# chem-rano/eigensolvers

Hardware: AMD Instinct MI355X
Metric: fp64 CSR SpMV GB/s (fused shift y = sigma*x - H x) (higher is better)
Workload: dtype f64; 1 GPU; random-sparse Hermitian CSR N=10000000 nnz/row~64 (BASELINE metric config), row-partitioned over 1 GPU(s); N=10000000, nnz=650007472, nnz_row_arg=64, kernel_variant=auto:column-window-blocked(workgroup), generator_seed=7, comm=auto

## Files before the change

### eigensolvers_amd/csrc/common.h

```cpp
#pragma once
#include <hip/hip_runtime.h>
#include <stdint.h>
#include <stdio.h>
#include <stdlib.h>
#include <string.h>
#include "../../include/hipeig.h"

#define HIPEIG_WAVE 64
#define HIPEIG_BLOCK 256
#define HIPEIG_MAX_PARTIALS 2048
#define HIPEIG_MAX_COLS 16
#define HIPEIG_WIDE_PARTIALS 32768
#define HIPEIG_GATHER_MAX_CHUNKS 4
#define HIPEIG_SLOT_DOUBLES 16
#define HIPEIG_MAX_RANKS 64

struct GatherLayout {
  int32_t nranks, nchunks;
  int64_t h;
  int64_t cbase[HIPEIG_GATHER_MAX_CHUNKS + 1];
  __host__ __device__ int64_t cstride(int c) const { return h + (c == nchunks - 1 ? HIPEIG_SLOT_DOUBLES : 0); }
  __host__ __device__ int64_t pos(int rank, int64_t i) const {
    int c = (int)(i / h);
    if (c >= nchunks) c = nchunks - 1;
// ... 86 lines not shown
  double* mr_ws;
  int64_t mr_ws_n;
  int64_t mr_ws_doubles;
  hipGraphExec_t mr_graph;
  void* mr_graph_key;
  size_t mr_graph_key_bytes;
  int use_graph;
  MinresState* d_mr_state;
  MinresState* h_mr_state;
  void* comm;
  void* loop;
  int nranks, rank;
  int collectives;
  int64_t mr_collectives;
  double* x_full;
  int64_t x_full_n;
  int64_t* row_counts;
  double* blk_ws;
  size_t blk_ws_doubles;
  double* xb_full;
  int64_t xb_full_n;
  double* mrb_ws;
  int64_t mrb_ws_n;
  MinresState* d_mrb_state;
  MinresState* h_mrb_state;
  double* mrbz_ws;
  int64_t mrbz_ws_n;
  int overlap;
  double* ytmp;
  int64_t ytmp_n;
  int gather_chunks;
  hipEvent_t ev_chunk[HIPEIG_GATHER_MAX_CHUNKS];
  unsigned* d_counters;
  double* d_group_partials;
  int phase_timing;
  hipEvent_t ev_ph[8];
  hipEvent_t ev_stage;
  hipEvent_t ev_slot[16];
  hipStream_t arn_stream[16];
  hipEvent_t ev_arn_in[16];
  int arn_nstreams;
  double* d_arn_ws;
  unsigned* d_arn_cnt;
  void* h_arn_items;
  void* d_arn_items;
  struct DirectComm* direct;
  int gather_backend;
  int allreduce_backend;
  int exchange_off;
  double* ms_ws;
  int64_t ms_ws_doubles;
  void* h_ms_state;
  double* lf_ws;
  int64_t lf_ws_doubles;
  void* h_lf_state;
  struct LfPoolEntry* lf_pool;
  int lf_pool_n, lf_pool_cap;
  int64_t lf_pool_bytes;
};

struct LfPoolEntry {
  double* p;
  size_t bytes;
};
void hipeig_lf_pool_clear(hipeig_ctx* c);
void arnoldi_release(hipeig_ctx* c);

struct BlockedLayout {
  uint32_t* idx;
  double* val;
  uint32_t* off;
  int32_t nunits, nwin, wbits, rw;
  int32_t wgs_per_sweep;
  int32_t csplit;
  int32_t binbits, align;
  int64_t slots;
  int32_t state;
};

static inline size_t blocked_lds_bytes(const BlockedLayout& L, int acc_per_row) {
  return (size_t)L.rw * acc_per_row * sizeof(double) + ((size_t)L.nwin + 2) * sizeof(uint32_t);
}

struct SweepGrid { int wgs, launches; };
static inline SweepGrid blocked_grid(const BlockedLayout& L, int units_per_wg = 1) {
  const int64_t total = L.csplit > 1 ? (int64_t)L.nunits * L.csplit : ((int64_t)L.nunits + units_per_wg - 1) / units_per_wg;
  int64_t g = (L.csplit > 1 || total < L.wgs_per_sweep) ? total : L.wgs_per_sweep;
  if (g < 1) g = 1;
  if (g > HIPEIG_MAX_PARTIALS) g = HIPEIG_MAX_PARTIALS;
  return SweepGrid{(int)g, (int)((total + g - 1) / g)};
}

enum : unsigned {
  BIN_LANE_MAJOR = 1,
  BIN_UNIT_BATCH = 2,
  BIN_GROUP_ALIGN = 4,
  BIN_WIN_BATCH = 8,
  BIN_UNCACHED = 16,
};

struct hipeig_csr {
  int64_t nrows, ncols, nnz, row_offset;
  int32_t* d_rowptr;
  int32_t* d_col;
  double* d_val;
  int32_t* d_row_blocks;
  int32_t n_row_blocks;
  BlockedLayout t;
  int32_t t_prefetch;
  BlockedLayout w;
  BlockedLayout p;
  BlockedLayout b[3];
  double* d_dense;
  int64_t dense_ld;
  int64_t dense_bytes;
  int32_t dense_grid_vec, dense_grid_blk;
  int32_t last_pair_fused;
  int reproducible;
  double absrow_max;
  int32_t block_variant;
  int32_t last_block_variant, last_block_k;
  int64_t gather_len;
  GatherLayout gl;
  RankRows rank_rows;
  int variant;
  int last_variant;
  int last_launches;
  int lanes_per_row;
  int64_t col_stride;
  int64_t bytes;
};

static inline int layout_slot(int K) { return K == 4 ? 0 : K == 8 ? 1 : 2; }

int hipeig_build_binned(hipeig_ctx* c, hipeig_csr* A, const BlockedLayout& geom, unsigned policy, BlockedLayout* out);
void hipeig_free_layout(BlockedLayout* L);

int hipeig_dense_refusal(const hipeig_ctx* c, const hipeig_csr* A);
int hipeig_dense_reserve(hipeig_ctx* c, hipeig_csr* A);
int hipeig_dense_grid(const hipeig_csr* A, int rows_per_wg);
void hipeig_dense_free(hipeig_csr* A);

int hipeig_sync_checked(hipeig_ctx* c);

int hipeig_comm_setup_rows(hipeig_ctx* ctx, int64_t nrows_local, GatherLayout* gl_out);
int hipeig_allreduce_sum(hipeig_ctx* ctx, double* d_buf, int count);
int hipeig_allgather_x(hipeig_ctx* ctx, const GatherLayout& gl, const double* x_local, int64_t n_local,
                       const double** x_full_out);
int hipeig_allgather_f64(hipeig_ctx* ctx, const double* send, double* recv, size_t count);
int hipeig_allgather_x_begin(hipeig_ctx* ctx, const GatherLayout& gl, const double* x_local, int64_t n_local);
int hipeig_allgather_x_wait_chunk(hipeig_ctx* ctx, const GatherLayout& gl, int chunk);
int hipeig_allgather_block(hipeig_ctx* ctx, const GatherLayout& gl, int K, const double* xb_local, int64_t n_local,
                           const double** xb_full_out);
double* hipeig_gather_slot(hipeig_ctx* ctx, const GatherLayout& gl);

__host__ __device__ __forceinline__ double mul_rn(double a, double b) {
#pragma clang fp contract(off)
  return a * b;
}
__host__ __device__ __forceinline__ double add_rn(double a, double b) {
#pragma clang fp contract(off)
  return a + b;
}

__device__ __forceinline__ double wave_reduce_sum(double v) {
#pragma unroll
  for (int off = 32; off > 0; off >>= 1) v += __shfl_down(v, off, 64);
  return v;
}

// ... 102 lines not shown
```

### eigensolvers_amd/csrc/spmv.hip

```cpp
#include <vector>
#include "sweep_launch.h"

static int build_tcoow_layout(hipeig_ctx* c, hipeig_csr* A, int pair);

struct AxpyEpilogue {
  double a_self, a_sum;
  const double* __restrict__ xl;
  double* __restrict__ y;
  __device__ __forceinline__ void row(int64_t r, double sum, double& acc) const {
    const double t = (a_self == 0.0) ? 0.0 : mul_rn(a_self, xl[r]);
    y[r] = add_rn(t, mul_rn(a_sum, sum));
  }
};

__global__ void __launch_bounds__(HIPEIG_BLOCK)
spmv_stream_kernel(CsrView A, const double* __restrict__ x, AxpyEpilogue epi) {
  __shared__ double prod[SPMV_NNZ_PER_BLOCK];
  double acc = 0.0;
  csr_stream_sweep(A, x, epi, acc, prod);
}

__global__ void __launch_bounds__(HIPEIG_BLOCK)
spmv_vector_kernel(CsrView A, const double* __restrict__ x, AxpyEpilogue epi) {
  double acc = 0.0;
  csr_vector_sweep(A, x, epi, acc);
}

__global__ void __launch_bounds__(HIPEIG_BLOCK)
spmv_tcoo_kernel(TcooView T, const double* __restrict__ x, AxpyEpilogue epi) {
  extern __shared__ double tcoo_lds[];
  double acc = 0.0;
  tcoo_sweep(T, x, epi, acc, tcoo_lds);
}

template <int FIXED>
__global__ void __launch_bounds__(TCOOW_THREADS)
spmv_tcoow_kernel(TcooView T, const double* __restrict__ x, AxpyEpilogue epi) {
  extern __shared__ double tcoo_lds[];
  __shared__ double red16[16];
  double acc = 0.0;
  tcoo_wg_sweep<AxpyEpilogue, FIXED>(T, x, epi, acc, tcoo_lds, red16);
}

__global__ void __launch_bounds__(HIPEIG_BLOCK)
spmv_dense_kernel(DenseView D, const double* __restrict__ x, AxpyEpilogue epi) {
  double acc = 0.0;
  dense_row_sweep(D, x, epi, acc);
}

struct PairEpilogue {
  double ar, ai, as;
  const double* __restrict__ xr;
  const double* __restrict__ xi;
  double* __restrict__ yr;
  double* __restrict__ yi;
  __device__ __forceinline__ void row2(int64_t r, double sr, double si, double& acc) const {
    const double vr = xr[r], vi = xi[r];
    const double tr = add_rn(mul_rn(ar, vr), mul_rn(as, sr));
    const double ti = add_rn(mul_rn(ar, vi), mul_rn(as, si));
    yr[r] = fma(-ai, vi, tr);
    yi[r] = fma(ai, vr, ti);
  }
};

__global__ void __launch_bounds__(TCOOW_THREADS)
spmv_tcoow_pair_kernel(TcooView T, const double* __restrict__ xpair, PairEpilogue epi) {
  extern __shared__ double tcoo_lds[];
  double acc = 0.0;
  tcoo_wg_sweep<PairEpilogue, 0, 1>(T, xpair, epi, acc, tcoo_lds, nullptr);
}

__global__ void __launch_bounds__(HIPEIG_BLOCK)
pair_pack_kernel(int64_t n, const double* __restrict__ xr, const double* __restrict__ xi, double2* __restrict__ xp) {
  const int64_t stride = (int64_t)gridDim.x * blockDim.x;
  for (int64_t i = (int64_t)blockIdx.x * blockDim.x + threadIdx.x; i < n; i += stride) xp[i] = make_double2(xr[i], xi[i]);
}

__global__ void __launch_bounds__(HIPEIG_BLOCK) absmax_kernel(const double* __restrict__ x, int64_t n, double* __restrict__ partials) {
  __shared__ double lds[16];
  double m = 0.0;
  const int64_t stride = (int64_t)gridDim.x * blockDim.x;
  for (int64_t i = (int64_t)blockIdx.x * blockDim.x + threadIdx.x; i < n; i += stride) {
    const double v = fabs(x[i]);
    m = (v > m || v != v) ? v : m;
// ... 3 lines not shown
}

__global__ void __launch_bounds__(HIPEIG_BLOCK)
rowabs_max_kernel(const int32_t* __restrict__ rowptr, const double* __restrict__ val, int64_t nrows, double* __restrict__ partials) {
  __shared__ double lds[16];
  const int lane = threadIdx.x & 63;
  const int64_t wave = ((int64_t)blockIdx.x * blockDim.x + threadIdx.x) >> 6;
  const int64_t nwaves = ((int64_t)gridDim.x * blockDim.x) >> 6;
  double m = 0.0;
  for (int64_t r = wave; r < nrows; r += nwaves) {
    double a = 0.0;
    for (int p = rowptr[r] + lane; p < rowptr[r + 1]; p += 64) a += fabs(val[p]);
    a = wave_reduce_sum(a);
    a = __shfl(a, 0, 64);
    m = fmax(m, a);
  }
  m = block_max_all(m, lds);
  if (threadIdx.x == 0) partials[blockIdx.x] = m;
}

__global__ void __launch_bounds__(HIPEIG_BLOCK) absmax_gathered_kernel(const double* __restrict__ x, GatherLayout gl, RankRows rows,
                                                                       double* __restrict__ partials) {
  __shared__ double lds[16];
  double m = 0.0;
  const int64_t stride = (int64_t)gridDim.x * blockDim.x, n = gl.total();
  for (int64_t p = (int64_t)blockIdx.x * blockDim.x + threadIdx.x; p < n; p += stride) {
    int k = 0;
    while (k + 1 < gl.nchunks && p >= gl.cbase[k + 1]) ++k;
    const int64_t q = p - gl.cbase[k], cs = gl.cstride(k);
    const int r = (int)(q / cs);
    const int64_t i = q - (int64_t)r * cs;
    if (i >= gl.h || (int64_t)k * gl.h + i >= rows.n[r]) continue;
    const double v = fabs(x[p]);
    m = (v > m || v != v) ? v : m;
  }
  m = block_max_all(m, lds);
  if (threadIdx.x == 0) partials[blockIdx.x] = m;
}

#define HIPEIG_FX_AREA (4 * HIPEIG_WIDE_PARTIALS)
int hipeig_fixed_prepare(hipeig_ctx* c, const hipeig_csr* A, const double* xg, TcooView* t) {
  const int g = grid_for(A->gather_len, 8);
  double* area = c->d_partials + HIPEIG_FX_AREA;
  if (A->col_stride > 0)
    hipLaunchKernelGGL(absmax_gathered_kernel, dim3(g), dim3(HIPEIG_BLOCK), 0, c->stream, xg, A->gl, A->rank_rows, area);
  else
    hipLaunchKernelGGL(absmax_kernel, dim3(g), dim3(HIPEIG_BLOCK), 0, c->stream, xg, A->gather_len, area);
  t->fx_xmax = area; t->fx_count = g; t->fx_bound = A->absrow_max;
  return 0;
}

__global__ void __launch_bounds__(HIPEIG_BLOCK)
spmv_tcoow_combine_kernel(const double* __restrict__ parts, int nparts, int64_t stride, int64_t nrows, AxpyEpilogue epi) {
  double acc = 0.0;
  tcoow_combine_sweep(parts, nparts, stride, nrows, epi, acc);
}

static auto spmv_launcher(hipeig_ctx* c, const SweepPlan& p, const AxpyEpilogue& epi) {
  const CsrView view = p.view;
  const DenseView dview = p.dview;
  return [=](auto v, auto f, int grid, int threads, size_t lds, const TcooView& tv, const double* xg, int) {
    constexpr int V = decltype(v)::value;
    const dim3 g(grid), t(threads);
    if constexpr (V == 6) hipLaunchKernelGGL(spmv_dense_kernel, g, t, lds, c->stream, dview, xg, epi);
    else if constexpr (V == 5) hipLaunchKernelGGL(spmv_tcoow_combine_kernel, g, t, lds, c->stream, tv.raw_out, tv.part_base, tv.part_stride, tv.nrows, epi);
    else if constexpr (V == 4) hipLaunchKernelGGL(spmv_tcoow_kernel<decltype(f)::value>, g, t, lds, c->stream, tv, xg, epi);
    else if constexpr (V == 3) hipLaunchKernelGGL(spmv_tcoo_kernel, g, t, lds, c->stream, tv, xg, epi);
    else if constexpr (V == 2) hipLaunchKernelGGL(spmv_stream_kernel, g, t, lds, c->stream, view, xg, epi);
    else hipLaunchKernelGGL(spmv_vector_kernel, g, t, lds, c->stream, view, xg, epi);
  };
}

TcooView hipeig_tcoo_view(const hipeig_csr* A, const BlockedLayout& L) {
  TcooView t;
  t.idx = L.idx; t.val = L.val; t.off = L.off;
  t.nunits = L.nunits; t.nwin = L.nwin; t.wbits = L.wbits; t.rw = L.rw;
  t.unit_begin = 0;
  t.prefetch = (&L == &A->t) ? A->t_prefetch : 0;
  t.ablate = 0;
  if (const char* e = getenv("HIPEIG_TCOO_ABLATE")) t.ablate = atoi(e);
  t.nrows = A->nrows;
  t.gather_len = A->gather_len;
  t.nrun = 0; t.yinit = nullptr; t.raw_out = nullptr;
  t.csplit = 1; t.part_base = 0; t.part_stride = 0;
  t.fx_xmax = nullptr; t.fx_count = 0; t.fx_bound = 0.0;
  return t;
}

CsrView hipeig_csr_view(const hipeig_csr* A) {
  CsrView v;
  v.rowptr = A->d_rowptr;
  v.col = A->d_col;
  v.val = A->d_val;
  v.row_blocks = A->d_row_blocks;
  v.n_row_blocks = A->n_row_blocks;
  v.nrows = A->nrows;
  v.group = A->lanes_per_row;
  return v;
}

SweepGrid hipeig_sweep_grid(const hipeig_csr* A, int variant) {
  if (variant == 6) return SweepGrid{hipeig_dense_grid(A, DENSE_ROWS_PER_WAVE * (HIPEIG_BLOCK / HIPEIG_WAVE)), 1};
  if (variant == 4 || variant == 5) return blocked_grid(A->w);
  if (variant == 3) return blocked_grid(A->t, 4);
  int64_t g = A->n_row_blocks;
  if (variant == 1) {
    const int64_t groups_per_block = HIPEIG_BLOCK / A->lanes_per_row;
    g = (A->nrows + groups_per_block - 1) / groups_per_block;
  }
  if (g < 1) g = 1;
  if (g > HIPEIG_MAX_PARTIALS) g = HIPEIG_MAX_PARTIALS;
  return SweepGrid{(int)g, 1};
}

static int tcoow_ensure_parts(hipeig_ctx* c, int64_t doubles) {
  if (c->ytmp_n >= doubles) return 0;
  if (c->ytmp) { if (hipFree(c->ytmp) != hipSuccess) return -1; }
  c->ytmp = nullptr; c->ytmp_n = 0;
  if (hipMalloc((void**)&c->ytmp, (size_t)doubles * sizeof(double)) != hipSuccess) {
    hipeig_set_error("out of device memory for the partial-sum slabs");
    return -1;
  }
  c->ytmp_n = doubles;
  return 0;
}

int64_t hipeig_tcoow_part_stride(const hipeig_csr* A) { return (A->nrows + 63) & ~(int64_t)63; }

struct WindowSets {
  int nset;
  int nrun[1 + HIPEIG_GATHER_MAX_CHUNKS];
  int lo[1 + HIPEIG_GATHER_MAX_CHUNKS][4], hi[1 + HIPEIG_GATHER_MAX_CHUNKS][4];
};

static void tcoow_window_sets(const hipeig_ctx* c, const hipeig_csr* A, WindowSets* ws) {
  const GatherLayout& gl = A->gl;
  const int wb = A->w.wbits, nwin = A->w.nwin;
  const int64_t W = (int64_t)1 << wb;
  memset(ws, 0, sizeof(*ws));
  ws->nset = 1 + gl.nchunks;
  int prev_end = 0;
  for (int k = 0; k < gl.nchunks; ++k) {
    int wend = (k == gl.nchunks - 1) ? nwin : (int)(gl.cbase[k + 1] >> wb);
    if (wend > nwin) wend = nwin;
    if (wend < prev_end) wend = prev_end;
    const int64_t rows_lo = (int64_t)k * gl.h;
    int64_t rows = A->nrows - rows_lo;
    if (rows > gl.h) rows = gl.h;
    int l0 = 0, l1 = 0;
    if (rows > 0) {
      const int64_t p0 = gl.cbase[k] + (int64_t)c->rank * gl.cstride(k), p1 = p0 + rows;
      l0 = (int)((p0 + W - 1) >> wb); l1 = (int)(p1 >> wb);
      if (l0 < prev_end) l0 = prev_end;
      if (l1 > wend) l1 = wend;
      if (l1 < l0) l1 = l0;
    }
    if (l1 > l0) {
      const int q = ws->nrun[0]++;
      ws->lo[0][q] = l0; ws->hi[0][q] = l1;
      if (l0 > prev_end) { const int r = ws->nrun[1 + k]++; ws->lo[1 + k][r] = prev_end; ws->hi[1 + k][r] = l0; }
      if (wend > l1) { const int r = ws->nrun[1 + k]++; ws->lo[1 + k][r] = l1; ws->hi[1 + k][r] = wend; }
    } else if (wend > prev_end) {
      const int r = ws->nrun[1 + k]++; ws->lo[1 + k][r] = prev_end; ws->hi[1 + k][r] = wend;
    }
    prev_end = wend;
  }
}
// ... 341 lines not shown
                         L.rw, L.binbits, (int)nbins, L.wbits, d_cur, idx, val, fill);
  };
  auto build = [&]() -> int {
    HIPEIG_CHECK(hipMalloc((void**)&d_cur, ncnt * sizeof(uint32_t)));
    HIPEIG_CHECK(hipMemsetAsync(d_cur, 0, ncnt * sizeof(uint32_t), c->stream));
    scatter(nullptr, nullptr, 0);
    HIPEIG_CHECK(hipGetLastError());
    std::vector<uint32_t> cnt(ncnt);
    HIPEIG_CHECK(hipMemcpyAsync(cnt.data(), d_cur, ncnt * sizeof(uint32_t), hipMemcpyDeviceToHost, c->stream));
    HIPEIG_CHECK(hipStreamSynchronize(c->stream));
    const bool unit_batch = policy & BIN_UNIT_BATCH, win_batch = policy & BIN_WIN_BATCH, align = L.align;
    std::vector<uint32_t> off(ntile + 1);
    uint64_t run = 0, counted = 0;
    for (size_t i = 0; i < ncnt; ++i) {
      if (i % bpw == 0) {
        const size_t tile = i / bpw;
        if ((unit_batch && tile % L.nwin == 0) || win_batch) run = (run + TCOOW_BATCH - 1) & ~(uint64_t)(TCOOW_BATCH - 1);
        else if (align) run = (run + 63) & ~(uint64_t)63;
        off[tile] = (uint32_t)run;
      }
      const uint32_t n = cnt[i];
      if (align && n > 0 && n <= 64 && (run & 63) + n > 64) run = (run + 63) & ~(uint64_t)63;
      cnt[i] = (uint32_t)run;
      run += n;
      counted += n;
    }
    off[ntile] = (uint32_t)run;
    HIPEIG_REQUIRE(counted == (uint64_t)A->nnz, "count pass lost non-zeros");
    if (unit_batch) run = (run + TCOOW_BATCH - 1) & ~(uint64_t)(TCOOW_BATCH - 1);
    HIPEIG_REQUIRE(run < ((uint64_t)1 << 32), "blocked stream too long for 32-bit offsets");
    L.slots = (int64_t)run;
    const size_t nslots = (size_t)run;
    HIPEIG_CHECK(hipMemcpyAsync(d_cur, cnt.data(), ncnt * sizeof(uint32_t), hipMemcpyHostToDevice, c->stream));
    HIPEIG_CHECK(hipMalloc((void**)&L.off, (ntile + 1) * sizeof(uint32_t)));
    if (policy & BIN_UNCACHED) {
      HIPEIG_CHECK(hipExtMallocWithFlags((void**)&L.idx, nslots * sizeof(uint32_t), hipDeviceMallocUncached));
      HIPEIG_CHECK(hipExtMallocWithFlags((void**)&L.val, nslots * sizeof(double), hipDeviceMallocUncached));
    } else {
      HIPEIG_CHECK(hipMalloc((void**)&L.idx, nslots * sizeof(uint32_t)));
      HIPEIG_CHECK(hipMalloc((void**)&L.val, nslots * sizeof(double)));
    }
    if (nslots != (size_t)A->nnz) {
      HIPEIG_CHECK(hipMemsetAsync(L.idx, 0xFF, nslots * sizeof(uint32_t), c->stream));
      HIPEIG_CHECK(hipMemsetAsync(L.val, 0, nslots * sizeof(double), c->stream));
    }
    HIPEIG_CHECK(hipMemcpyAsync(L.off, off.data(), (ntile + 1) * sizeof(uint32_t), hipMemcpyHostToDevice, c->stream));
    scatter(L.idx, L.val, 1);
    HIPEIG_CHECK(hipGetLastError());
    HIPEIG_CHECK(hipStreamSynchronize(c->stream));
    return 0;
  };
  const int rc = build();
  if (d_cur) hipFree(d_cur);
  if (rc) { hipeig_free_layout(&L); return rc; }
  *out = L;
  A->bytes += L.slots * 12 + (int64_t)(ntile + 1) * 4;
  return 0;
}

static int build_tcoow_layout(hipeig_ctx* c, hipeig_csr* A, int pair) {
  BlockedLayout& out = pair ? A->p : A->w;
  if (out.idx) return 0;
  if (A->nnz == 0 || A->nrows == 0) return 2;
  const int acc = pair ? 2 : 1;
  const int64_t max_rw = TCOOW_MAX_RW / acc;
  int wbits = 17;
  if (const char* e = getenv(pair ? "HIPEIG_TCOOW_PAIR_WBITS" : "HIPEIG_TCOOW_WBITS")) wbits = atoi(e);
  HIPEIG_REQUIRE(wbits >= 10 && wbits <= 17, "HIPEIG_TCOOW_WBITS out of range");
  while (wbits > 10 && ((int64_t)1 << (wbits - 1)) >= A->gather_len) --wbits;
  const int nwin = (int)((A->gather_len + ((int64_t)1 << wbits) - 1) >> wbits);
  if (nwin > TCOOW_MAX_WIN) return 2;
  int binbits = 4;
  if (const char* e = getenv(pair ? "HIPEIG_TCOOW_PAIR_BINBITS" : "HIPEIG_TCOOW_BINBITS")) binbits = atoi(e);
  if (binbits > wbits) binbits = wbits;
  HIPEIG_REQUIRE(binbits >= 3, "HIPEIG_TCOOW_BINBITS out of range");
  int64_t sweeps = (A->nrows + (int64_t)c->num_cu * max_rw - 1) / ((int64_t)c->num_cu * max_rw);
  if (sweeps < 1) sweeps = 1;
  int64_t rw = (A->nrows + sweeps * c->num_cu - 1) / (sweeps * c->num_cu);
  rw = (rw + 63) / 64 * 64;
  if (rw < 64) rw = 64;
  if (rw > max_rw) rw = max_rw;
  int csplit = 1;
  if (!pair) {
    const int64_t rb_min = (A->nrows + TCOOW_MAX_RW - 1) / TCOOW_MAX_RW;
    int want = (rb_min * 2 <= c->num_cu && A->gather_len >= 4000000) ? (int)(c->num_cu / rb_min) : 1;
    if (const char* e = getenv("HIPEIG_TCOOW_CSPLIT")) want = atoi(e);
    if (want > 64) want = 64;
    if (want > 1 && rb_min * want <= HIPEIG_MAX_PARTIALS) {
      csplit = want;
      rw = ((A->nrows + rb_min - 1) / rb_min + 63) / 64 * 64;
      if (rw > TCOOW_MAX_RW) rw = TCOOW_MAX_RW;
    }
  }
  if (const char* e = getenv(pair ? "HIPEIG_TCOOW_PAIR_RW" : "HIPEIG_TCOOW_RW")) rw = (atoi(e) + 63) / 64 * 64;
  HIPEIG_REQUIRE(rw >= 64 && rw <= max_rw && rw < ((int64_t)1 << (32 - wbits)), "HIPEIG_TCOOW_RW out of range");
  BlockedLayout G{};
  G.nunits = (int)((A->nrows + rw - 1) / rw); G.nwin = nwin; G.wbits = wbits; G.rw = (int)rw;
  G.binbits = binbits; G.csplit = csplit;
  int per_cu = (int)(163840 / (blocked_lds_bytes(G, acc) + 256));
  if (per_cu > 2) per_cu = 2;
  if (per_cu < 1) per_cu = 1;
  if (const char* e = getenv("HIPEIG_TCOOW_WG_PER_LAUNCH_CU")) per_cu = atoi(e);
  HIPEIG_REQUIRE(per_cu >= 1 && per_cu <= 8, "HIPEIG_TCOOW_WG_PER_LAUNCH_CU out of range");
  G.wgs_per_sweep = per_cu * c->num_cu;
  const char* al_env = getenv(pair ? "HIPEIG_TCOOW_PAIR_ALIGN" : "HIPEIG_TCOOW_ALIGN");
  const char* uc = getenv("HIPEIG_TCOOW_UNCACHED");
  const unsigned policy = BIN_LANE_MAJOR | BIN_UNIT_BATCH | (al_env && atoi(al_env) == 0 ? 0u : BIN_GROUP_ALIGN) |
                          (A->col_stride > 0 ? BIN_WIN_BATCH : 0u) | (uc && atoi(uc) != 0 ? BIN_UNCACHED : 0u);
  const int rc = hipeig_build_binned(c, A, G, policy, &out);
  if (rc) return rc;
  if (pair) {
    HIPEIG_CHECK(hipFuncSetAttribute((const void*)spmv_tcoow_pair_kernel, hipFuncAttributeMaxDynamicSharedMemorySize,
                                     (int)HIPEIG_TCOOW_LDS_MAX));
    return 0;
  }
  HIPEIG_CHECK(hipFuncSetAttribute((const void*)spmv_tcoow_kernel<0>, hipFuncAttributeMaxDynamicSharedMemorySize,
                                   (int)HIPEIG_TCOOW_LDS_MAX));
  HIPEIG_CHECK(hipFuncSetAttribute((const void*)spmv_tcoow_kernel<1>, hipFuncAttributeMaxDynamicSharedMemorySize,
                                   (int)HIPEIG_TCOOW_LDS_MAX));
  {
    const int gr = 8 * c->num_cu < HIPEIG_MAX_PARTIALS ? 8 * c->num_cu : HIPEIG_MAX_PARTIALS;
    double* area = c->d_partials + HIPEIG_FX_AREA;
    hipLaunchKernelGGL(rowabs_max_kernel, dim3(gr), dim3(HIPEIG_BLOCK), 0, c->stream, A->d_rowptr, A->d_val, A->nrows, area);
    std::vector<double> part((size_t)gr);
    HIPEIG_CHECK(hipMemcpyAsync(part.data(), area, sizeof(double) * gr, hipMemcpyDeviceToHost, c->stream));
    HIPEIG_CHECK(hipStreamSynchronize(c->stream));
    double m = 0.0;
    for (double v : part) m = (v > m || v != v) ? v : m;
    A->absrow_max = m;
  }
  return 0;
}

int hipeig_csr_build_tcoow(hipeig_ctx* c, hipeig_csr* A) { return build_tcoow_layout(c, A, 0); }

int hipeig_csr_pick_variant(hipeig_ctx* c, hipeig_csr* A) {
  int variant = A->variant;
  if (variant == 6 && hipeig_dense_reserve(c, A)) return -1;
  if (variant == 0) {
    variant = (A->gather_len * 8 > (int64_t)3 << 20 && A->nnz > (int64_t)1 << 20) ? (A->reproducible ? 5 : 4) : 2;
  }
  if (variant == 4 || variant == 5) {
    const int rc = hipeig_csr_build_tcoow(c, A);
    if (rc == 1) return -1;
    if (rc == 2) variant = 3;
  }
  if (variant == 3) {
    const int rc = hipeig_csr_build_tcoo(c, A);
    if (rc == 1) return -1;
    if (rc == 2) variant = 2;
  }
  A->last_variant = variant;
  A->last_launches = hipeig_sweep_grid(A, variant).launches;
  return variant;
}

__global__ void remap_cols_kernel(int32_t* __restrict__ col, int64_t nnz, const int64_t* __restrict__ offs,
                                  GatherLayout gl) {
  const int64_t step = (int64_t)gridDim.x * blockDim.x;
  for (int64_t p = (int64_t)blockIdx.x * blockDim.x + threadIdx.x; p < nnz; p += step) {
    const int64_t j = col[p];
    int lo = 0, hi = gl.nranks - 1;
    while (lo < hi) {
      const int mid = (lo + hi + 1) >> 1;
      if (j >= offs[mid]) lo = mid; else hi = mid - 1;
    }
    col[p] = (int32_t)gl.pos(lo, j - offs[lo]);
  }
}

int hipeig_csr_finalize(hipeig_ctx* c, hipeig_csr* A, const int32_t* rowptr32) {
  std::vector<int32_t> rb;
  rb.reserve((size_t)(A->nnz / (SPMV_NNZ_PER_BLOCK / 2) + 16));
  rb.push_back(0);
// ... 154 lines not shown
```

### eigensolvers_amd/csrc/spmv_device.h

```cpp
#pragma once
#include "common.h"

#define SPMV_NNZ_PER_BLOCK 2048
#define SPMV_PER_THREAD (SPMV_NNZ_PER_BLOCK / HIPEIG_BLOCK)

struct CsrView {
  const int32_t* __restrict__ rowptr;
  const int32_t* __restrict__ col;
  const double* __restrict__ val;
  const int32_t* __restrict__ row_blocks;
  int32_t n_row_blocks;
  int64_t nrows;
  int group;
};

__device__ __forceinline__ double group_reduce_sum(double v, int group) {
  for (int off = group >> 1; off > 0; off >>= 1) v += __shfl_down(v, off, group);
  return v;
}

template <class Epi>
__device__ __forceinline__ void csr_stream_sweep(const CsrView& A, const double* __restrict__ x,
                                                 const Epi& epi, double& acc, double* prod ) {
  const int tid = threadIdx.x;
// ... 8 lines not shown
      int cidx[SPMV_PER_THREAD];
      double v[SPMV_PER_THREAD];
#pragma unroll
      for (int u = 0; u < SPMV_PER_THREAD; ++u) {
        const int k = tid + u * HIPEIG_BLOCK;
        if (k < nn) {
          cidx[u] = __builtin_nontemporal_load(A.col + p0 + k);
          v[u] = __builtin_nontemporal_load(A.val + p0 + k);
        }
      }
#pragma unroll
      for (int u = 0; u < SPMV_PER_THREAD; ++u) {
        const int k = tid + u * HIPEIG_BLOCK;
        if (k < nn) v[u] *= x[cidx[u]];
      }
#pragma unroll
      for (int u = 0; u < SPMV_PER_THREAD; ++u) {
        const int k = tid + u * HIPEIG_BLOCK;
        if (k < nn) prod[k] = v[u];
      }
      __syncthreads();
      for (int r = r0 + gid; r < r1; r += ngroups) {
        const int s = A.rowptr[r] - p0, e = A.rowptr[r + 1] - p0;
        double sum = 0.0;
        for (int k = s + glane; k < e; k += group) sum += prod[k];
        sum = group_reduce_sum(sum, group);
        if (glane == 0) epi.row(r, sum, acc);
      }
      __syncthreads();
    } else {
      double sum = 0.0;
      for (int p = p0 + tid; p < p1; p += HIPEIG_BLOCK)
        sum = fma(__builtin_nontemporal_load(A.val + p), x[__builtin_nontemporal_load(A.col + p)], sum);
      sum = block_reduce_sum(sum, prod);
      if (tid == 0) epi.row(r0, sum, acc);
    }
  }
}

template <class Epi>
__device__ __forceinline__ void csr_vector_sweep(const CsrView& A, const double* __restrict__ x,
                                                 const Epi& epi, double& acc) {
  const int group = A.group;
  const int64_t gid = ((int64_t)blockIdx.x * HIPEIG_BLOCK + threadIdx.x) / group;
  const int glane = threadIdx.x % group;
  const int64_t ngroups = (int64_t)gridDim.x * HIPEIG_BLOCK / group;
  for (int64_t r = gid; r < A.nrows; r += ngroups) {
    const int s = A.rowptr[r], e = A.rowptr[r + 1];
    double sum = 0.0;
    for (int p = s + glane; p < e; p += group)
      sum = fma(__builtin_nontemporal_load(A.val + p), x[__builtin_nontemporal_load(A.col + p)], sum);
    sum = group_reduce_sum(sum, group);
    if (glane == 0) epi.row(r, sum, acc);
  }
}

#define TCOO_MAX_WBITS 18
#define TCOO_MAX_RW 2560
#define TCOO_MAX_WIN 128
#define HIPEIG_TCOO_LDS_MAX ((size_t)4 * TCOO_MAX_RW * sizeof(double))
#ifndef TCOO_UNROLL
#define TCOO_UNROLL 4
#endif

#ifdef HIPEIG_EXPERIMENTS
#define TCOO_ABL(T, bit) ((T).ablate & (bit))
#else
#define TCOO_ABL(T, bit) 0
#endif

struct TcooView {
  const uint32_t* __restrict__ idx;
  const double* __restrict__ val;
  const uint32_t* __restrict__ off;
  int32_t nunits, nwin, wbits, rw;
  int32_t unit_begin;
  int32_t prefetch;
  int32_t ablate;
  int64_t nrows, gather_len;
  int32_t nrun;
  int32_t run_lo[4], run_hi[4];
  const double* yinit;
  double* raw_out;
  int32_t csplit, part_base;
  int64_t part_stride;
  const double* fx_xmax;
  int32_t fx_count;
  double fx_bound;
};

__device__ __forceinline__ void lds_add_f64(double* p, double v) {
  __hip_atomic_fetch_add(p, v, __ATOMIC_RELAXED, __HIP_MEMORY_SCOPE_WAVEFRONT);
}

__device__ __forceinline__ double tcoo_prefetch_window(const double* __restrict__ x, int64_t gather_len,
                                                       int c, int wbits, int lane, int wid, int wpb) {
  const int64_t w0 = (int64_t)c << wbits;
  int64_t wlen = (int64_t)1 << wbits;
  if (w0 + wlen > gather_len) wlen = gather_len - w0;
  if (wlen <= 0) return 0.0;
  const int nslices = ((gridDim.x + 7) / 8) * wpb;
  const int rank = (blockIdx.x / 8) * wpb + wid;
  int64_t per = ((wlen + nslices - 1) / nslices + 15) & ~(int64_t)15;
  const int64_t s0 = (int64_t)rank * per;
  int64_t s1 = s0 + per;
  if (s1 > wlen) s1 = wlen;
  double pf = 0.0;
  const double* base = x + w0;
  for (int64_t i = s0 + 2 * lane; i + 1 < s1; i += 128) {
    const double2 t = *reinterpret_cast<const double2*>(base + i);
    pf += t.x + t.y;
  }
  return pf;
}

template <class Epi>
__device__ __forceinline__ void tcoo_sweep(const TcooView& T, const double* __restrict__ x, const Epi& epi,
                                           double& acc, double* lds ) {
  const int lane = threadIdx.x & 63, wid = threadIdx.x >> 6;
  const int waves_per_block = blockDim.x >> 6;
  double* yacc = lds + (size_t)wid * T.rw;
  const uint32_t cmask = (1u << T.wbits) - 1u;
  const int u = T.unit_begin + blockIdx.x * waves_per_block + wid;
  double pf = 0.0;
  if (T.prefetch) pf += tcoo_prefetch_window(x, T.gather_len, 0, T.wbits, lane, wid, waves_per_block);
  if (u < T.nunits) {
    for (int k = lane; k < T.rw; k += 64) yacc[k] = 0.0;
    const uint32_t* offu = T.off + (size_t)u * T.nwin;
    uint32_t end = offu[0];
    for (int c = 0; c < T.nwin; ++c) {
      const uint32_t beg = end;
      end = offu[c + 1];
      if (T.prefetch && c + 1 < T.nwin)
        pf += tcoo_prefetch_window(x, T.gather_len, c + 1, T.wbits, lane, wid, waves_per_block);
      const double* __restrict__ xw = x + ((size_t)c << T.wbits);
      for (uint32_t base = beg; base < end; base += 64 * TCOO_UNROLL) {
        uint32_t id[TCOO_UNROLL];
        double v[TCOO_UNROLL];
#pragma unroll
        for (int j = 0; j < TCOO_UNROLL; ++j) {
          const uint32_t q = base + lane + 64 * j;
          const bool ok = q < end;
          id[j] = ok ? __builtin_nontemporal_load(T.idx + q) : 0xFFFFFFFFu;
          v[j] = ok ? __builtin_nontemporal_load(T.val + q) : 0.0;
        }
        if (!(TCOO_ABL(T, 1))) {
#pragma unroll
          for (int j = 0; j < TCOO_UNROLL; ++j)
            if (id[j] != 0xFFFFFFFFu) v[j] *= xw[id[j] & cmask];
        }
        if (!(TCOO_ABL(T, 2))) {
#pragma unroll
          for (int j = 0; j < TCOO_UNROLL; ++j)
            if (id[j] != 0xFFFFFFFFu) lds_add_f64(yacc + (id[j] >> T.wbits), v[j]);
        } else {
#pragma unroll
          for (int j = 0; j < TCOO_UNROLL; ++j) pf += v[j] + (double)id[j];
        }
      }
    }
    const int64_t r0 = (int64_t)u * T.rw;
    for (int k = lane; k < T.rw && r0 + k < T.nrows; k += 64) epi.row(r0 + k, yacc[k], acc);
  }
  asm volatile("" ::"v"(pf));
}

#ifndef TCOOW_THREADS
#define TCOOW_THREADS 1024
#endif
#define TCOOW_MAX_RW 20224
#define TCOOW_MAX_WIN 256
#define HIPEIG_TCOOW_LDS_MAX ((size_t)TCOOW_MAX_RW * sizeof(double) + (TCOOW_MAX_WIN + 2) * sizeof(uint32_t))

#define TCOOW_BATCH 256
#if defined(TCOOW_INTERLEAVE) && TCOOW_INTERLEAVE
#error "TCOOW_INTERLEAVE (waves on adjacent 64-element groups) does not match the lane-major TCOO-W stream"
#endif
__host__ __device__ __forceinline__ uint32_t tcoow_islot(uint32_t s) {
  return (s & ~255u) | ((s & 63u) << 2) | ((s >> 6) & 3u);
}
__host__ __device__ __forceinline__ uint32_t tcoow_vslot(uint32_t s) {
  return (s & ~255u) | ((s & 128u) >> 0) | ((s & 63u) << 1) | ((s >> 6) & 1u);
}
typedef uint32_t tcoow_u32x4 __attribute__((ext_vector_type(4)));
typedef double tcoow_f64x2 __attribute__((ext_vector_type(2)));

__device__ __forceinline__ void lds_add_f64_wg(double* p, double v) {
  __hip_atomic_fetch_add(p, v, __ATOMIC_RELAXED, __HIP_MEMORY_SCOPE_WORKGROUP);
}

#ifndef TCOOW_GATHER_MODE
#define TCOOW_GATHER_MODE 0
#endif
#ifndef TCOOW_GIF
#define TCOOW_GIF 1
#endif
__device__ __forceinline__ double tcoow_gather(const double* p) {
#if TCOOW_GATHER_MODE == 1
  return __builtin_nontemporal_load(p);
#elif TCOOW_GATHER_MODE == 2
  return __hip_atomic_load(p, __ATOMIC_RELAXED, __HIP_MEMORY_SCOPE_AGENT);
#elif TCOOW_GATHER_MODE == 3
  return __hip_atomic_load(p, __ATOMIC_RELAXED, __HIP_MEMORY_SCOPE_SYSTEM);
#else
  return *p;
#endif
}

template <class Epi>
__device__ __forceinline__ void tcoow_combine_sweep(const double* __restrict__ parts, int nparts, int64_t stride,
                                                    int64_t nrows, const Epi& epi, double& acc) {
  const int64_t step = (int64_t)gridDim.x * blockDim.x;
  for (int64_t r = (int64_t)blockIdx.x * blockDim.x + threadIdx.x; r < nrows; r += step) {
    double s = parts[r];
    for (int p = 1; p < nparts; ++p) s += parts[(int64_t)p * stride + r];
    epi.row(r, s, acc);
  }
}

__device__ __forceinline__ double block_max_all(double v, double* lds) {
#pragma unroll
  for (int off = 32; off > 0; off >>= 1) v = fmax(v, __shfl_xor(v, off, 64));
  const int lane = threadIdx.x & 63, wid = threadIdx.x >> 6;
  if (lane == 0) lds[wid] = v;
  __syncthreads();
  double r = lds[0];
  for (int w = 1; w < (int)(blockDim.x >> 6); ++w) r = fmax(r, lds[w]);
  __syncthreads();
  return r;
}

__device__ __forceinline__ double fixed_point_scale(double bound, double xmax) {
  const double v = bound * xmax;
  if (!(v > 0.0)) return (v == 0.0) ? 1.0 : __builtin_nan("");
  if (!(v < 1.7976931348623157e308)) return __builtin_nan("");
  int ex;
  frexp(v, &ex);
  int e = 61 - ex;
  e = e > 1000 ? 1000 : (e < -1000 ? -1000 : e);
  return ldexp(1.0, e);
}

__device__ __forceinline__ void lds_add_i64_wg(double* slot, double scaled) {
  __hip_atomic_fetch_add(reinterpret_cast<unsigned long long*>(slot), (unsigned long long)__double2ll_rn(scaled),
                         __ATOMIC_RELAXED, __HIP_MEMORY_SCOPE_WORKGROUP);
}

template <class Epi, int FIXED = 0, int PAIR = 0>
__device__ __forceinline__ void tcoo_wg_sweep(const TcooView& T, const double* __restrict__ x, const Epi& epi,
                                              double& acc, double* yacc ,
                                              double* red16 = nullptr ) {
  static_assert(!(FIXED && PAIR), "the pair sweep has no fixed-point form");
  const int lane = threadIdx.x & 63, wid = threadIdx.x >> 6;
  const int nw = blockDim.x >> 6;
  const uint32_t cmask = (1u << T.wbits) - 1u;
  const int vb = T.unit_begin + blockIdx.x;
  const int u = (T.csplit > 1) ? vb / T.csplit : vb;
  const int cs = (T.csplit > 1) ? vb - u * T.csplit : 0;
  if (u >= T.nunits) return;
  uint32_t* offL = reinterpret_cast<uint32_t*>(yacc + (PAIR ? 2 : 1) * T.rw);
  const int64_t r0 = (int64_t)u * T.rw;
  double fx_scale = 1.0, fx_inv = 1.0;
  if (FIXED) {
    double m = 0.0;
    for (int k = threadIdx.x; k < T.fx_count; k += blockDim.x) m = fmax(m, T.fx_xmax[k]);
    m = block_max_all(m, red16);
    fx_scale = fixed_point_scale(T.fx_bound, m);
    fx_inv = 1.0 / fx_scale;
  }
  if (PAIR) {
    for (int k = threadIdx.x; k < 2 * T.rw; k += blockDim.x) yacc[k] = 0.0;
  } else {
    for (int k = threadIdx.x; k < T.rw; k += blockDim.x) {
      const double y0 = (T.yinit && r0 + k < T.nrows) ? T.yinit[r0 + k] : 0.0;
      if (FIXED) reinterpret_cast<long long*>(yacc)[k] = __double2ll_rn(y0 * fx_scale);
      else yacc[k] = y0;
    }
  }
  for (int k = threadIdx.x; k <= T.nwin; k += blockDim.x) offL[k] = T.off[(size_t)u * T.nwin + k];
  __syncthreads();
  const uint32_t step = (uint32_t)nw * 64 * TCOO_UNROLL;
  static_assert(TCOO_UNROLL == 4, "the lane-major stream of the TCOO-W layout holds 4 elements per lane and batch");
  const uint32_t jstride = 64;
  const uint32_t wave_off = (uint32_t)wid * 64 * TCOO_UNROLL;
  int c = 0;
  double sink = 0.0;
  uint32_t idA[TCOO_UNROLL], idB[TCOO_UNROLL];
  double vA[TCOO_UNROLL], vB[TCOO_UNROLL];
#define TCOO_LOAD(ID, V, BASE)                                                         \
  {                                                                                    \
     \
     \
    const uint32_t bl = (TCOO_ABL(T, 16)) ? sbeg + (((BASE) - sbeg) & 4095u) : (BASE);  \
     \
     \
    const tcoow_u32x4 iv = __builtin_nontemporal_load(reinterpret_cast<const tcoow_u32x4*>(T.idx + (size_t)bl + 4 * lane)); \
    tcoow_f64x2 v01 = {1.0, 1.0}, v23 = {1.0, 1.0};                                   \
    if (!(TCOO_ABL(T, 4))) {                                                           \
      const double* vb = T.val + (size_t)bl + 2 * lane;                                \
      v01 = __builtin_nontemporal_load(reinterpret_cast<const tcoow_f64x2*>(vb));       \
      v23 = __builtin_nontemporal_load(reinterpret_cast<const tcoow_f64x2*>(vb + 128)); \
    }                                                                                  \
    ID[0] = iv.x; ID[1] = iv.y; ID[2] = iv.z; ID[3] = iv.w;                            \
    V[0] = v01.x; V[1] = v01.y; V[2] = v23.x; V[3] = v23.y;                            \
  }
#define TCOO_CONSUME(ID, V, BASE)                                                      \
  {                                                                                    \
    int cw[TCOO_UNROLL];                                                               \
    _Pragma("unroll") for (int j = 0; j < TCOO_UNROLL; ++j) {                          \
      const uint32_t q = (BASE) + lane + jstride * j;                                       \
      if (!(q < send)) ID[j] = 0xFFFFFFFFu;           \
       \
       \
      while (q < send && c + 1 < T.nwin && q >= offL[c + 1]) ++c;                      \
      cw[j] = c;                                                                       \
    }                                                                                  \
    double V2[TCOO_UNROLL];                                                            \
    if (TCOOW_GIF > 1 && !PAIR) {                                                      \
       \
       \
      double xg[TCOO_UNROLL];                                                          \
      _Pragma("unroll") for (int j = 0; j < TCOO_UNROLL; ++j) {                        \
        const size_t gi = (ID[j] != 0xFFFFFFFFu) ? ((size_t)cw[j] << T.wbits) + (ID[j] & cmask) : 0; \
        xg[j] = tcoow_gather(x + gi);                                                  \
      }                                                                                \
      _Pragma("unroll") for (int j = 0; j < TCOO_UNROLL; ++j) V[j] *= xg[j];           \
    } else if (!(TCOO_ABL(T, 1))) {                                                      \
      _Pragma("unroll") for (int j = 0; j < TCOO_UNROLL; ++j)                          \
        if (ID[j] != 0xFFFFFFFFu) {                                                    \
          const size_t gi = ((size_t)((TCOO_ABL(T, 8)) ? 0 : cw[j]) << T.wbits) + (ID[j] & cmask); \
          if (PAIR) {                                                                  \
            const double2 xv = *reinterpret_cast<const double2*>(x + 2 * gi);          \
            V2[j] = V[j] * xv.y;                                                       \
            V[j] *= xv.x;                                                              \
          } else {                                                                     \
            V[j] *= tcoow_gather(x + gi);                                              \
          }                                                                            \
        }                                                                              \
    } else if (PAIR) {                                                                 \
      _Pragma("unroll") for (int j = 0; j < TCOO_UNROLL; ++j) V2[j] = V[j];            \
    }                                                                                  \
// ... 63 lines not shown
```

### eigensolvers_amd/csrc/sweep_launch.h

```cpp
#pragma once
#include <type_traits>
#include "spmv_device.h"
#include "dense_device.h"

CsrView hipeig_csr_view(const hipeig_csr* A);
TcooView hipeig_tcoo_view(const hipeig_csr* A, const BlockedLayout& L);
int hipeig_tcoow_reserve(hipeig_ctx* c, const hipeig_csr* A);
SweepGrid hipeig_sweep_grid(const hipeig_csr* A, int variant);
int hipeig_csr_pick_variant(hipeig_ctx* c, hipeig_csr* A);
size_t hipeig_tcoo_lds_bytes(const hipeig_csr* A);
DenseView hipeig_dense_view(const hipeig_csr* A);
void hipeig_phase_mark(hipeig_ctx* c, int k);
const double* hipeig_gathered(hipeig_ctx* c);

struct SweepPlan {
  int variant;
  int fixed;
  CsrView view;
  TcooView tview;
  DenseView dview;
  size_t lds;
  int gA, nsweep;
  bool split;
  int gC;
  int nPA;
};

static inline int sweep_plan_build(hipeig_ctx* c, hipeig_csr* A, int combine_grid, SweepPlan* p) {
  p->variant = hipeig_csr_pick_variant(c, A);
  if (p->variant < 0) return 1;
  p->fixed = (p->variant == 5) ? 1 : 0;
  if (p->fixed) p->variant = 4;
  HIPEIG_REQUIRE((p->variant >= 1 && p->variant <= 4) || p->variant == 6, "unknown sweep layout");
  if (p->variant == 4 && hipeig_tcoow_reserve(c, A)) return 1;
  p->view = hipeig_csr_view(A);
  p->tview = hipeig_tcoo_view(A, (p->variant == 4) ? A->w : A->t);
  p->dview = hipeig_dense_view(A);
  p->lds = (p->variant == 4) ? blocked_lds_bytes(A->w, 1) : (p->variant == 3) ? hipeig_tcoo_lds_bytes(A) : 0;
  const SweepGrid sg = hipeig_sweep_grid(A, p->variant);
  p->gA = sg.wgs; p->nsweep = sg.launches;
  p->split = (p->variant == 4) && A->w.csplit > 1;
  p->gC = combine_grid;
  p->nPA = p->split ? p->gC : p->gA * p->nsweep;
  if (p->variant == 6) A->dense_grid_vec = p->gA;
  return 0;
}

static inline int sweep_set_lds_limits(const SweepPlan& p, const void* k3, const void* k40, const void* k41) {
  if (p.variant == 3) HIPEIG_CHECK(hipFuncSetAttribute(k3, hipFuncAttributeMaxDynamicSharedMemorySize, (int)HIPEIG_TCOO_LDS_MAX));
  if (p.variant == 4) {
    HIPEIG_CHECK(hipFuncSetAttribute(k40, hipFuncAttributeMaxDynamicSharedMemorySize, (int)HIPEIG_TCOOW_LDS_MAX));
    HIPEIG_CHECK(hipFuncSetAttribute(k41, hipFuncAttributeMaxDynamicSharedMemorySize, (int)HIPEIG_TCOOW_LDS_MAX));
  }
  return 0;
}

struct SweepOperand {
  const double* xg;
  TcooView tv;
  bool has_last;
  int ncombine;
};

int hipeig_tcoow_run_plan(hipeig_ctx* c, hipeig_csr* A, const SweepPlan& p, const double* x_local, SweepOperand* o);

static inline int sweep_prepare(hipeig_ctx* c, hipeig_csr* A, const SweepPlan& p, const double* x_local, SweepOperand* o) {
  o->xg = nullptr; o->tv = p.tview; o->has_last = true; o->ncombine = 0;
  if (p.variant == 4) return hipeig_tcoow_run_plan(c, A, p, x_local, o) ? 4 : 0;
  if (p.variant == 6) { o->xg = x_local; return 0; }
  return hipeig_allgather_x(c, A->gl, x_local, A->nrows, &o->xg) ? 4 : 0;
}

template <class Launch>
static inline void sweep_launch(hipeig_ctx* c, const SweepPlan& p, const SweepOperand& o, Launch&& launch) {
  using std::integral_constant;
  TcooView tv = o.tv;
  if (p.variant == 4) {
    if (o.has_last) {
      for (int sw = 0; sw < p.nsweep; ++sw) {
        tv.unit_begin = sw * p.gA;
        if (p.fixed) launch(integral_constant<int, 4>{}, integral_constant<int, 1>{}, p.gA, TCOOW_THREADS, p.lds, tv, o.xg, sw * p.gA);
        else launch(integral_constant<int, 4>{}, integral_constant<int, 0>{}, p.gA, TCOOW_THREADS, p.lds, tv, o.xg, sw * p.gA);
      }
    }
    if (o.ncombine) {
      tv.raw_out = c->ytmp;
      tv.part_base = o.ncombine;
      launch(integral_constant<int, 5>{}, integral_constant<int, 0>{}, p.gC, HIPEIG_BLOCK, (size_t)0, tv, o.xg, 0);
    }
  } else if (p.variant == 3) {
    for (int sw = 0; sw < p.nsweep; ++sw) {
      tv.unit_begin = sw * p.gA * 4;
      launch(integral_constant<int, 3>{}, integral_constant<int, 0>{}, p.gA, HIPEIG_BLOCK, p.lds, tv, o.xg, sw * p.gA);
    }
  } else if (p.variant == 6) {
    launch(integral_constant<int, 6>{}, integral_constant<int, 0>{}, p.gA, HIPEIG_BLOCK, (size_t)0, tv, o.xg, 0);
  } else if (p.variant == 1) {
    launch(integral_constant<int, 1>{}, integral_constant<int, 0>{}, p.gA, HIPEIG_BLOCK, (size_t)0, tv, o.xg, 0);
  } else {
    launch(integral_constant<int, 2>{}, integral_constant<int, 0>{}, p.gA, HIPEIG_BLOCK, (size_t)0, tv, o.xg, 0);
  }
}
```

Before: 4351 GB/s.

## Pick TCOOW row-block/column-split shape via cost model and XCD-aware workgroup mapping

Replaces the fixed column-split heuristic with a cost model that scans row-block counts and split factors. It estimates per-nnz cycles from x-window reuse (expected hits per window) plus the cost of the extra partial traffic, and only switches away from the old choice when the estimate clears a tie margin. Split grids are now capped by the partial-buffer size and run as several launches of a fixed number of units. Workgroups are remapped with a modulo-8 interleave so consecutive work items land on the same chiplet, which is meant to improve L2 locality. The risk is that a miscalibrated model picks a worse shape, and the grid padding adds idle workgroups.

```diff
diff --git a/eigensolvers_amd/csrc/common.h b/eigensolvers_amd/csrc/common.h
--- a/eigensolvers_amd/csrc/common.h
+++ b/eigensolvers_amd/csrc/common.h
@@ -192,10 +192,17 @@
   return (size_t)L.rw * acc_per_row * sizeof(double) + ((size_t)L.nwin + 2) * sizeof(uint32_t);
 }
 
-struct SweepGrid { int wgs, launches; };
+struct SweepGrid { int wgs, launches, units = 0; };
 static inline SweepGrid blocked_grid(const BlockedLayout& L, int units_per_wg = 1) {
-  const int64_t total = L.csplit > 1 ? (int64_t)L.nunits * L.csplit : ((int64_t)L.nunits + units_per_wg - 1) / units_per_wg;
-  int64_t g = (L.csplit > 1 || total < L.wgs_per_sweep) ? total : L.wgs_per_sweep;
+  if (L.csplit > 1) {
+    static_assert(HIPEIG_MAX_PARTIALS % 8 == 0, "a split grid is rounded up to 8 under the cap");
+    int64_t units = HIPEIG_MAX_PARTIALS / L.csplit;
+    if (units > L.nunits) units = L.nunits;
+    if (units < 1) units = 1;
+    return SweepGrid{(int)((units * L.csplit + 7) / 8 * 8), (int)((L.nunits + units - 1) / units), (int)units};
+  }
+  const int64_t total = ((int64_t)L.nunits + units_per_wg - 1) / units_per_wg;
+  int64_t g = (total < L.wgs_per_sweep) ? total : L.wgs_per_sweep;
   if (g < 1) g = 1;
   if (g > HIPEIG_MAX_PARTIALS) g = HIPEIG_MAX_PARTIALS;
   return SweepGrid{(int)g, (int)((total + g - 1) / g)};
diff --git a/eigensolvers_amd/csrc/spmv.hip b/eigensolvers_amd/csrc/spmv.hip
--- a/eigensolvers_amd/csrc/spmv.hip
+++ b/eigensolvers_amd/csrc/spmv.hip
@@ -1,5 +1,6 @@
 #include <vector>
 #include "sweep_launch.h"
+#include "tcoow_shape.h"
 
 static int build_tcoow_layout(hipeig_ctx* c, hipeig_csr* A, int pair);
 
@@ -169,7 +170,7 @@
   t.nrows = A->nrows;
   t.gather_len = A->gather_len;
   t.nrun = 0; t.yinit = nullptr; t.raw_out = nullptr;
-  t.csplit = 1; t.part_base = 0; t.part_stride = 0;
+  t.csplit = 1; t.part_base = 0; t.part_stride = 0; t.launch_units = 0;
   t.fx_xmax = nullptr; t.fx_count = 0; t.fx_bound = 0.0;
   return t;
 }
@@ -677,14 +678,17 @@
   if (rw > max_rw) rw = max_rw;
   int csplit = 1;
   if (!pair) {
-    const int64_t rb_min = (A->nrows + TCOOW_MAX_RW - 1) / TCOOW_MAX_RW;
-    int want = (rb_min * 2 <= c->num_cu && A->gather_len >= 4000000) ? (int)(c->num_cu / rb_min) : 1;
-    if (const char* e = getenv("HIPEIG_TCOOW_CSPLIT")) want = atoi(e);
-    if (want > 64) want = 64;
-    if (want > 1 && rb_min * want <= HIPEIG_MAX_PARTIALS) {
-      csplit = want;
-      rw = ((A->nrows + rb_min - 1) / rb_min + 63) / 64 * 64;
-      if (rw > TCOOW_MAX_RW) rw = TCOOW_MAX_RW;
+    if (const char* e = getenv("HIPEIG_TCOOW_CSPLIT")) {
+      const int64_t rb_min = (A->nrows + TCOOW_MAX_RW - 1) / TCOOW_MAX_RW;
+      int want = atoi(e);
+      if (want > 64) want = 64;
+      if (want > 1 && rb_min * want <= HIPEIG_MAX_PARTIALS) {
+        csplit = want;
+        rw = tcoow_rows_per_block(A->nrows, rb_min, TCOOW_MAX_RW);
+      }
+    } else {
+      const TcoowShape s = tcoow_pick_shape(A->nrows, A->nnz, A->gather_len, c->num_cu, TCOOW_MAX_RW, HIPEIG_MAX_PARTIALS);
+      if (s.splits > 1) { csplit = s.splits; rw = s.rw; }
     }
   }
   if (const char* e = getenv(pair ? "HIPEIG_TCOOW_PAIR_RW" : "HIPEIG_TCOOW_RW")) rw = (atoi(e) + 63) / 64 * 64;
diff --git a/eigensolvers_amd/csrc/spmv_device.h b/eigensolvers_amd/csrc/spmv_device.h
--- a/eigensolvers_amd/csrc/spmv_device.h
+++ b/eigensolvers_amd/csrc/spmv_device.h
@@ -114,7 +114,7 @@
   int32_t run_lo[4], run_hi[4];
   const double* yinit;
   double* raw_out;
-  int32_t csplit, part_base;
+  int32_t csplit, part_base, launch_units;
   int64_t part_stride;
   const double* fx_xmax;
   int32_t fx_count;
@@ -278,6 +278,17 @@
                          __ATOMIC_RELAXED, __HIP_MEMORY_SCOPE_WORKGROUP);
 }
 
+__host__ __device__ __forceinline__ int tcoow_item_of_workgroup(int b, int grid, int items) {
+  const int x = b & 7, j = b >> 3;
+  if ((grid & 7) == 0 && grid >= items) {
+    const int lo = (x * items + 7) >> 3, hi = ((x + 1) * items + 7) >> 3;
+    return lo + j < hi ? lo + j : -1;
+  }
+  const int q = grid >> 3, r = grid & 7;
+  const int item = x * q + (x < r ? x : r) + j;
+  return item < items ? item : -1;
+}
+
 template <class Epi, int FIXED = 0, int PAIR = 0>
 __device__ __forceinline__ void tcoo_wg_sweep(const TcooView& T, const double* __restrict__ x, const Epi& epi,
                                               double& acc, double* yacc ,
@@ -286,9 +297,13 @@
   const int lane = threadIdx.x & 63, wid = threadIdx.x >> 6;
   const int nw = blockDim.x >> 6;
   const uint32_t cmask = (1u << T.wbits) - 1u;
-  const int vb = T.unit_begin + blockIdx.x;
-  const int u = (T.csplit > 1) ? vb / T.csplit : vb;
-  const int cs = (T.csplit > 1) ? vb - u * T.csplit : 0;
+  int u = T.unit_begin + blockIdx.x, cs = 0;
+  if (T.csplit > 1) {
+    const int item = tcoow_item_of_workgroup(blockIdx.x, gridDim.x, T.launch_units * T.csplit);
+    if (item < 0) return;
+    cs = item / T.launch_units;
+    u = T.unit_begin + (item - cs * T.launch_units);
+  }
   if (u >= T.nunits) return;
   uint32_t* offL = reinterpret_cast<uint32_t*>(yacc + (PAIR ? 2 : 1) * T.rw);
   const int64_t r0 = (int64_t)u * T.rw;
diff --git a/eigensolvers_amd/csrc/sweep_launch.h b/eigensolvers_amd/csrc/sweep_launch.h
--- a/eigensolvers_amd/csrc/sweep_launch.h
+++ b/eigensolvers_amd/csrc/sweep_launch.h
@@ -21,6 +21,7 @@
   DenseView dview;
   size_t lds;
   int gA, nsweep;
+  int uA;
   bool split;
   int gC;
   int nPA;
@@ -38,7 +39,7 @@
   p->dview = hipeig_dense_view(A);
   p->lds = (p->variant == 4) ? blocked_lds_bytes(A->w, 1) : (p->variant == 3) ? hipeig_tcoo_lds_bytes(A) : 0;
   const SweepGrid sg = hipeig_sweep_grid(A, p->variant);
-  p->gA = sg.wgs; p->nsweep = sg.launches;
+  p->gA = sg.wgs; p->nsweep = sg.launches; p->uA = sg.units;
   p->split = (p->variant == 4) && A->w.csplit > 1;
   p->gC = combine_grid;
   p->nPA = p->split ? p->gC : p->gA * p->nsweep;
@@ -79,6 +80,10 @@
     if (o.has_last) {
       for (int sw = 0; sw < p.nsweep; ++sw) {
         tv.unit_begin = sw * p.gA;
+        if (tv.csplit > 1) {
+          tv.unit_begin = sw * p.uA;
+          tv.launch_units = (tv.nunits - tv.unit_begin < p.uA) ? tv.nunits - tv.unit_begin : p.uA;
+        }
         if (p.fixed) launch(integral_constant<int, 4>{}, integral_constant<int, 1>{}, p.gA, TCOOW_THREADS, p.lds, tv, o.xg, sw * p.gA);
         else launch(integral_constant<int, 4>{}, integral_constant<int, 0>{}, p.gA, TCOOW_THREADS, p.lds, tv, o.xg, sw * p.gA);
       }
diff --git a/eigensolvers_amd/csrc/tcoow_shape.h b/eigensolvers_amd/csrc/tcoow_shape.h
--- /dev/null
+++ b/eigensolvers_amd/csrc/tcoow_shape.h
@@ -0,0 +1,61 @@
+#pragma once
+#include <cmath>
+#include <cstdint>
+
+struct TcoowShape {
+  int32_t nrb;
+  int32_t splits;
+  int32_t rw;
+};
+
+static const double TCOOW_SHAPE_TIE = 108.0 / 115.0;
+static const double TCOOW_SHAPE_CLOCK_HZ = 2.4e9;
+static const double TCOOW_SHAPE_STREAM_BPS = 5.8e12;
+static const int64_t TCOOW_SHAPE_MIN_GATHER = 4000000;
+static const int TCOOW_SHAPE_MAX_SPLITS = 64;
+
+static inline double tcoow_cycles_per_nnz(double k) {
+  const double f = k > 1e-9 ? (1.0 - std::exp(-k)) / k : 1.0;
+  return f * 2.6 + (1.0 - f) * 0.67 + 12.0 / 64.0;
+}
+
+static inline int64_t tcoow_rows_per_block(int64_t nrows, int64_t nrb, int64_t max_rw) {
+  int64_t rw = ((nrows + nrb - 1) / nrb + 63) / 64 * 64;
+  return rw > max_rw ? max_rw : rw;
+}
+
+static inline double tcoow_shape_cost(int64_t nrows, double nnz_row, int64_t ncols, int num_cu, int64_t max_rw,
+                                      int64_t nrb, int s, int64_t* rw_out, int64_t* units_out) {
+  const int64_t rw = tcoow_rows_per_block(nrows, nrb, max_rw);
+  const int64_t units = (nrows + rw - 1) / rw;
+  const int64_t items = units * s;
+  const double k = 16.0 * (double)rw * nnz_row / (double)ncols;
+  const double passes = (double)((items + num_cu - 1) / num_cu);
+  double cost = passes * tcoow_cycles_per_nnz(k) / (double)items;
+  if (s > 1) cost += (double)s * 16.0 / nnz_row * TCOOW_SHAPE_CLOCK_HZ / TCOOW_SHAPE_STREAM_BPS;
+  *rw_out = rw; *units_out = units;
+  return cost;
+}
+
+static inline TcoowShape tcoow_pick_shape(int64_t nrows, int64_t nnz, int64_t ncols, int num_cu, int64_t max_rw, int64_t max_partials) {
+  TcoowShape none{0, 1, 0};
+  if (nrows <= 0 || nnz <= 0 || ncols <= 0 || num_cu <= 0) return none;
+  const int64_t rb_min = (nrows + max_rw - 1) / max_rw;
+  if (rb_min > num_cu || ncols < TCOOW_SHAPE_MIN_GATHER) return none;
+  const double nnz_row = (double)nnz / (double)nrows;
+  int64_t rw, units;
+  const int s0 = (rb_min * 2 <= num_cu) ? (int)(num_cu / rb_min > TCOOW_SHAPE_MAX_SPLITS ? TCOOW_SHAPE_MAX_SPLITS : num_cu / rb_min) : 1;
+  const int64_t nrb0 = (s0 > 1) ? rb_min : num_cu;
+  double best = tcoow_shape_cost(nrows, nnz_row, ncols, num_cu, max_rw, nrb0, s0, &rw, &units);
+  TcoowShape pick = (s0 > 1 && rb_min * s0 <= max_partials) ? TcoowShape{(int32_t)units, s0, (int32_t)rw} : none;
+  if (pick.splits == 1 && s0 > 1) best = tcoow_shape_cost(nrows, nnz_row, ncols, num_cu, max_rw, num_cu, 1, &rw, &units);
+  double bar = best * TCOOW_SHAPE_TIE;
+  for (int64_t nrb = rb_min; nrb <= num_cu; ++nrb) {
+    int s = (int)(num_cu / nrb);
+    if (s > TCOOW_SHAPE_MAX_SPLITS) s = TCOOW_SHAPE_MAX_SPLITS;
+    if (s < 2 || nrb * s > max_partials) continue;
+    const double cost = tcoow_shape_cost(nrows, nnz_row, ncols, num_cu, max_rw, nrb, s, &rw, &units);
+    if (cost < bar) { bar = cost; pick = TcoowShape{(int32_t)units, s, (int32_t)rw}; }
+  }
+  return pick;
+}
```

Result: no change. 4351 GB/s (median of 2 runs) (-0.0%).
